# val-iisc/Reflecting-Reality

Hardware: AMD Instinct MI355X
Metric: images/sec at 512x512, 50-step DDIM, SD1.5+BrushNet (higher is better)
Workload: dtype bf16; 1 GPU; SD1.5 + BrushNet(6 cond ch) depth-cond inpaint, batch 4x512x512 per GPU, 50-step DDIM, CFG 7.5, VAE encode+decode included, random-init weights, inputs resident on the device; per_gpu_batch=4, global_batch=4, height=512, width=512, denoise_steps=50, parallelism=batch-shard x1 (no collective)

## Files before the change

reflecting-reality_amd/csrc/gemm_pers.hip:

```cpp
#include <hip/hip_runtime.h>

#include "gemm_conv_kernel.h"

namespace mfgemm {

namespace {

constexpr int PB_BM = 128, PB_BN = 160, PB_STAGES = 3, PB_PF = PB_STAGES - 1;
constexpr int PB_STAGE_BYTES = (PB_BM + PB_BN) * 128;
constexpr int PB_SLAB_RS = PB_BN * 2 + 16;
constexpr int PB_SLAB_OFF = PB_STAGES * PB_STAGE_BYTES;
constexpr int PB_SLAB_RST = PB_BM * 2 + 16;
constexpr int PB_SLAB_BYTES = PB_BN * PB_SLAB_RST;
static_assert(PB_SLAB_BYTES >= PB_BM * PB_SLAB_RS, "the slab region holds either layout");
constexpr int PB_LNST_OFF = PB_SLAB_OFF + PB_SLAB_BYTES;
constexpr int PB_EROW_OFF = PB_LNST_OFF + PB_BM * 8;
constexpr int PB_EROW_BYTES = 2 * PB_BN * 4;
constexpr int PB_LUT_OFF = PB_EROW_OFF + 2 * PB_EROW_BYTES;
constexpr int PB_LUT_N = 768;
constexpr int PB_SMEM = PB_LUT_OFF;
constexpr int PB_SMEM_GEGLU = PB_LUT_OFF + PB_LUT_N * 8;
static_assert(PB_SMEM_GEGLU <= 160 * 1024, "LDS");
constexpr int PB_CPR = PB_BN / 8;
constexpr int PB_CHUNKS = PB_BM * PB_CPR / 64;
constexpr int PB_CE = 6, PB_CC = 2;
static_assert(4 * PB_CE + 8 * PB_CC == PB_CHUNKS, "chunk ownership covers the slab");

template <bool F16, bool RES, bool GEGLU>
__device__ __forceinline__ void pers_item(const GemmArgs& p, int m, int n, const char* sp, const uint4& q, const char* lut) {
    const uint4 s = *reinterpret_cast<const uint4*>(sp);
    if constexpr (GEGLU) {
        float v[8], g[4];
        unpack_h8<F16>(s, v);
#pragma unroll
        for (int j = 0; j < 4; ++j) {
            const float x = v[4 + j];
            const float u = fmaf(__builtin_amdgcn_fmed3f(x, -6.0f, 5.984375f), 64.0f, 384.0f);
            const float fr = __builtin_amdgcn_fractf(u);
            const float2 e = *reinterpret_cast<const float2*>(lut + (int)(u - fr) * 8);
            g[j] = v[j] * (x * fmaf(fr, e.y, e.x));
        }
        uint2 u;
        u.x = pack_h2<F16>(g[0], g[1]);
        u.y = pack_h2<F16>(g[2], g[3]);
        *reinterpret_cast<uint2*>(p.out + ((int64_t)m * p.ldc + (n >> 1)) * 2) = u;
    } else {
        uint4 o = s;
        if (RES || p.act == MF_ACT_SILU) {
            float v[8];
            unpack_h8<F16>(s, v);
            if constexpr (RES) {
                float r[8];
                unpack_h8<F16>(q, r);
#pragma unroll
                for (int j = 0; j < 8; ++j) v[j] += r[j];
            }
            if (p.act == MF_ACT_SILU) {
#pragma unroll
                for (int j = 0; j < 8; ++j) v[j] = silu_precise(v[j]);
            }
            o = pack_h8<F16>(v);
        }
        *reinterpret_cast<uint4*>(p.out + ((int64_t)m * p.ldc + n) * 2) = o;
    }
}

__device__ __forceinline__ void pers_item_vt(const GemmArgs& p, int m, int n, const char* sp) {
    const uint4 s = *reinterpret_cast<const uint4*>(sp);
    const int img = m / p.vt_tokens, tok = m - img * p.vt_tokens;
    *reinterpret_cast<uint4*>(p.vt_out + (((int64_t)img * (p.N - p.vt_n0) + (n - p.vt_n0)) * p.vt_ld + tok) * 2) = s;
}

template <int DT, bool RES, bool GEGLU, bool LN, bool VT>
__global__ __launch_bounds__(1024) void gemm_pers_kernel(const GemmArgs p) {
    extern __shared__ __attribute__((aligned(16))) char smem[];
    constexpr bool F16 = DT == MF_F16;
    const int tid = (int)threadIdx.x, wave = __builtin_amdgcn_readfirstlane(tid >> 6), lane = tid & 63;
    const int role = wave < 8 ? 0 : (wave < 12 ? 1 : 2), rw = role == 0 ? wave : (wave & 3);
    int bid = (int)blockIdx.x;
    {
        const int nblk = (int)gridDim.x, q = nblk >> 3, r = nblk & 7, x = bid & 7, j = bid >> 3;
        bid = (x < r ? x * (q + 1) : r * (q + 1) + (x - r) * q) + j;
    }
    const int range = bid / p.tiles_m, tile_m = bid - range * p.tiles_m;
    const int m0 = tile_m * PB_BM, nt0 = range * p.nloop;
    const int nkt = p.nkt, G = p.nloop * nkt;
    const unsigned lds0 = __builtin_amdgcn_readfirstlane((unsigned)(size_t)(lds_ptr_t)smem);
    float2* lnst = reinterpret_cast<float2*>(smem + PB_LNST_OFF);
    const int dbg = p.dbg_epi;

    if constexpr (GEGLU) {
        if (tid < PB_LUT_N) {
            const float x0 = -6.0f + (float)tid * 0.015625f, x1 = x0 + 0.015625f;
            const float p0 = 0.5f * erfcf(-x0 * 0.70710678118654752440f), p1 = 0.5f * erfcf(-x1 * 0.70710678118654752440f);
            *reinterpret_cast<float2*>(smem + PB_LUT_OFF + tid * 8) = make_float2(p0, p1 - p0);
        }
        __builtin_amdgcn_s_waitcnt(0xc07f);
    }

    auto item_coords = [&](int c, int& row, int& cg) {
        int it = c * 64 + lane;
        asm volatile("" : "+v"(it));
        row = it / PB_CPR;
        cg = it - row * PB_CPR;
    };
    auto do_chunk = [&](int c, int n0, const uint4& qv) {
        if (VT && n0 >= p.vt_n0) {
            int it = c * 64 + lane;
            asm volatile("" : "+v"(it));
            const int col = it >> 4, rg = it & 15;
            pers_item_vt(p, m0 + rg * 8, n0 + col, smem + PB_SLAB_OFF + col * PB_SLAB_RST + rg * 16);
            return;
        }
        int row, cg;
        item_coords(c, row, cg);
        uint4 q = qv;
        if constexpr (RES) asm volatile("" : "+v"(q.x), "+v"(q.y), "+v"(q.z), "+v"(q.w));
        pers_item<F16, RES, GEGLU>(p, m0 + row, n0 + cg * 8, smem + PB_SLAB_OFF + row * PB_SLAB_RS + cg * 16, q, smem + PB_LUT_OFF);
    };
    auto fetch_res = [&](int c, int n0) -> uint4 {
        int row, cg;
        item_coords(c, row, cg);
        return *reinterpret_cast<const uint4*>(p.res0 + ((int64_t)(m0 + row) * p.ld_res0 + n0 + cg * 8) * 2);
    };

    if ((GEGLU || (dbg & 16)) && role == 0) __builtin_amdgcn_s_setprio(1);
    if ((dbg & 32) && role == 1) __builtin_amdgcn_s_setprio(1);
    if ((dbg & 64) && role == 2) __builtin_amdgcn_s_setprio(1);
    if (role == 1) {
        const srd_t sA = make_srd(p.a0, (unsigned)((int64_t)p.M * p.ld0b));
        const srd_t sW = make_srd(p.w, (unsigned)(((int64_t)(p.N - 1) * p.ldw + p.K) * 2));
        const int r8 = lane >> 3, slot = lane & 7;
        unsigned offA[4], offW[5];
#pragma unroll
        for (int i = 0; i < 4; ++i) {
            const int r = (4 * rw + i) * 8 + r8;
            offA[i] = (unsigned)(m0 + r) * (unsigned)p.ld0b + (unsigned)((slot ^ ((r >> 1) & 7)) << 4);
        }
#pragma unroll
        for (int i = 0; i < 5; ++i) {
            const int r = (5 * rw + i) * 8 + r8;
            offW[i] = (unsigned)(nt0 * PB_BN + r) * (unsigned)(p.ldw * 2) + (unsigned)((slot ^ ((r >> 1) & 7)) << 4);
        }
        const unsigned wstep = (unsigned)PB_BN * (unsigned)(p.ldw * 2);
        int i_kt = 0, i_st = 0;
        unsigned wbase = 0;
        const bool nodma = (dbg & 4) != 0;
        auto issue = [&]() {
            const unsigned ldsS = lds0 + i_st * PB_STAGE_BYTES;
            if (!nodma) {
#pragma unroll
                for (int i = 0; i < 4; ++i) dma16_buf(offA[i] + i_kt * 128, sA, ldsS + ((4 * rw + i) * 8) * 128);
#pragma unroll
                for (int i = 0; i < 5; ++i) dma16_buf(offW[i] + wbase + i_kt * 128, sW, ldsS + PB_BM * 128 + ((5 * rw + i) * 8) * 128);
            }
            i_st = i_st == PB_STAGES - 1 ? 0 : i_st + 1;
            if (++i_kt == nkt) { i_kt = 0; wbase += wstep; }
        };
        auto wait_newer = [&](int newer) {
            if (newer >= 2) wait_vmcnt<18>();
            else if (newer == 1) wait_vmcnt<9>();
            else wait_vmcnt<0>();
        };
        static_assert(PB_PF <= 2, "wait_newer covers 0 .. 2 younger tiles");
        for (int k = 0; k < PB_PF && k < G; ++k) issue();
        wait_newer((G < PB_PF ? G : PB_PF) - 1);
        __builtin_amdgcn_s_barrier();
        for (int g = 0; g + 1 < G; ++g) {
            if (g + PB_PF < G) issue();
            const int youngest = g + PB_PF < G ? g + PB_PF : G - 1;
            wait_newer(youngest - (g + 1));
            __builtin_amdgcn_s_barrier();
        }
        __builtin_amdgcn_s_barrier();
    } else if (role == 0) {
        const int wm = rw >> 1, wn = rw & 1, r16 = lane & 15, kg = lane >> 4;
        const int key16 = (r16 >> 1) & 7;
        f32x4_t acc[2][5];
#pragma unroll
        for (int a = 0; a < 2; ++a)
#pragma unroll
            for (int b = 0; b < 5; ++b) acc[a][b] = f32x4_t{0.0f, 0.0f, 0.0f, 0.0f};
        auto dump_vt = [&](int jt) {
            const char* er = smem + PB_EROW_OFF + (jt & 1) * PB_EROW_BYTES;
            const float alpha = p.alpha;
            const int odd = r16 & 1;
            float2 rst[2];
            if constexpr (LN) {
#pragma unroll
                for (int a = 0; a < 2; ++a) rst[a] = lnst[wm * 32 + 16 * a + r16];
            }
#pragma unroll
            for (int b = 0; b < 5; ++b) {
                const int col = wn * 80 + 16 * b + 4 * kg;
                const float4 bias = *reinterpret_cast<const float4*>(er + col * 4);
                float4 cs = make_float4(0, 0, 0, 0);
                if constexpr (LN) cs = *reinterpret_cast<const float4*>(er + PB_BN * 4 + col * 4);
#pragma unroll
                for (int a = 0; a < 2; ++a) {
                    float x[4] = {acc[a][b][0], acc[a][b][1], acc[a][b][2], acc[a][b][3]};
                    if constexpr (LN) {
                        x[0] = rst[a].y * (x[0] - rst[a].x * cs.x); x[1] = rst[a].y * (x[1] - rst[a].x * cs.y);
                        x[2] = rst[a].y * (x[2] - rst[a].x * cs.z); x[3] = rst[a].y * (x[3] - rst[a].x * cs.w);
                    }
                    x[0] = (x[0] + bias.x) * alpha; x[1] = (x[1] + bias.y) * alpha; x[2] = (x[2] + bias.z) * alpha; x[3] = (x[3] + bias.w) * alpha;
                    const float s0 = odd ? x[0] : x[2], s1 = odd ? x[1] : x[3];
                    const float g0 = __builtin_bit_cast(float, __builtin_amdgcn_mov_dpp(__builtin_bit_cast(int, s0), 0xB1, 0xF, 0xF, true));
                    const float g1 = __builtin_bit_cast(float, __builtin_amdgcn_mov_dpp(__builtin_bit_cast(int, s1), 0xB1, 0xF, 0xF, true));
                    const uint32_t d0 = pack_h2<F16>(odd ? g0 : x[0], odd ? x[2] : g0);
                    const uint32_t d1 = pack_h2<F16>(odd ? g1 : x[1], odd ? x[3] : g1);
                    char* sp = smem + PB_SLAB_OFF + (col + 2 * odd) * PB_SLAB_RST + (wm * 32 + 16 * a + (r16 & ~1)) * 2;
                    *reinterpret_cast<uint32_t*>(sp) = d0;
                    *reinterpret_cast<uint32_t*>(sp + PB_SLAB_RST) = d1;
                    acc[a][b] = f32x4_t{0.0f, 0.0f, 0.0f, 0.0f};
                }
            }
        };
        auto dump_plain = [&](int jt) {
            const char* er = smem + PB_EROW_OFF + (jt & 1) * PB_EROW_BYTES;
            const float alpha = p.alpha;
            float2 rst[2];
            if constexpr (LN) {
#pragma unroll
                for (int a = 0; a < 2; ++a) rst[a] = lnst[wm * 32 + 16 * a + r16];
            }
#pragma unroll
            for (int b = 0; b < 5; ++b) {
                const int col = wn * 80 + 16 * b + 4 * kg;
                const float4 bias = *reinterpret_cast<const float4*>(er + col * 4);
                float4 cs = make_float4(0, 0, 0, 0);
                if constexpr (LN) cs = *reinterpret_cast<const float4*>(er + PB_BN * 4 + col * 4);
#pragma unroll
                for (int a = 0; a < 2; ++a) {
                    float x[4] = {acc[a][b][0], acc[a][b][1], acc[a][b][2], acc[a][b][3]};
                    if constexpr (LN) {
                        x[0] = rst[a].y * (x[0] - rst[a].x * cs.x); x[1] = rst[a].y * (x[1] - rst[a].x * cs.y);
                        x[2] = rst[a].y * (x[2] - rst[a].x * cs.z); x[3] = rst[a].y * (x[3] - rst[a].x * cs.w);
                    }
                    x[0] = (x[0] + bias.x) * alpha; x[1] = (x[1] + bias.y) * alpha; x[2] = (x[2] + bias.z) * alpha; x[3] = (x[3] + bias.w) * alpha;
                    uint2 h;
                    h.x = pack_h2<F16>(x[0], x[1]);
                    h.y = pack_h2<F16>(x[2], x[3]);
                    *reinterpret_cast<uint2*>(smem + PB_SLAB_OFF + (wm * 32 + 16 * a + r16) * PB_SLAB_RS + col * 2) = h;
                    acc[a][b] = f32x4_t{0.0f, 0.0f, 0.0f, 0.0f};
                }
            }
        };
        auto is_vt = [&](int jt) -> bool { return VT && (nt0 + jt) * PB_BN >= p.vt_n0; };
        auto dump = [&](int jt) {
            if (is_vt(jt)) dump_vt(jt);
            else dump_plain(jt);
        };
        uint4 q[RES ? PB_CC : 1];
        auto prefetch = [&](int jt) {
            if constexpr (RES) {
                const int n0 = (nt0 + jt) * PB_BN;
#pragma unroll
                for (int i = 0; i < PB_CC; ++i) q[i] = fetch_res(4 * PB_CE + PB_CC * rw + i, n0);
            }
        };
        if (p.nloop > 1) prefetch(0);
        const int avail = nkt - 1, per = (PB_CC + avail - 1) / avail;
        int st = 0, kt = 0, jt = 0, pend_n0 = -1, done = 0;
        const bool nomma = (dbg & 2) != 0;
        __builtin_amdgcn_s_barrier();
        for (int g = 0; g < G; ++g) {
            const bool dumping = kt == 0 && g > 0;
            if (dumping && !(dbg & 8)) dump(jt - 1);
            if (!nomma) {
                const char* A16 = smem + st * PB_STAGE_BYTES + (wm * 32 + r16) * 128;
                const char* B16 = smem + st * PB_STAGE_BYTES + PB_BM * 128 + (wn * 80 + r16) * 128;
                uint4 fa[2][2], fb[2][5];
#pragma unroll
                for (int ks = 0; ks < 2; ++ks) {
#pragma unroll
                    for (int a = 0; a < 2; ++a) fa[ks][a] = *reinterpret_cast<const uint4*>(A16 + a * 16 * 128 + (((4 * ks + kg) ^ key16) << 4));
#pragma unroll
                    for (int b = 0; b < 5; ++b) fb[ks][b] = *reinterpret_cast<const uint4*>(B16 + b * 16 * 128 + (((4 * ks + kg) ^ key16) << 4));
                }
#pragma unroll
                for (int ks = 0; ks < 2; ++ks)
#pragma unroll
                    for (int a = 0; a < 2; ++a)
#pragma unroll
                        for (int b = 0; b < 5; ++b)
                            acc[a][b] = mfma16x32<DT>(__builtin_bit_cast(bf16x8_t, fb[ks][b]), __builtin_bit_cast(bf16x8_t, fa[ks][a]), acc[a][b], 0, 0, 0);
            }
            st = st == PB_STAGES - 1 ? 0 : st + 1;
            if (pend_n0 >= 0 && !dumping) {
                if (done == 0) {
                    if constexpr (RES) {
                        asm volatile("s_waitcnt vmcnt(0)" ::: "memory");
#pragma unroll
                        for (int i = 0; i < PB_CC; ++i) asm volatile("" : "+v"(q[i].x), "+v"(q[i].y), "+v"(q[i].z), "+v"(q[i].w));
                    }
                }
#pragma unroll 1
                for (int i = 0; i < per && done < PB_CC; ++i, ++done) {
                    if (dbg & 1) continue;
                    if (done == 0) do_chunk(4 * PB_CE + PB_CC * rw, pend_n0, q[0]);
                    else do_chunk(4 * PB_CE + PB_CC * rw + 1, pend_n0, q[RES ? 1 : 0]);
                }
                if (done == PB_CC) {
                    pend_n0 = -1;
                    if (jt < p.nloop - 1) prefetch(jt);
                }
            }
            if (dumping) { pend_n0 = (nt0 + jt - 1) * PB_BN; done = 0; }
            if (++kt == nkt) { kt = 0; ++jt; }
            __builtin_amdgcn_s_waitcnt(0xc07f);
            __builtin_amdgcn_s_barrier();
        }
        dump(p.nloop - 1);
        __builtin_amdgcn_s_waitcnt(0xc07f);
    } else {
        uint4 q[RES ? PB_CE : 1];
        float4 pb = make_float4(0, 0, 0, 0), pc = make_float4(0, 0, 0, 0);
        constexpr bool rows_duty = true;
        auto prefetch = [&](int jt) {
            if constexpr (RES) {
                const int n0 = (nt0 + jt) * PB_BN;
#pragma unroll
                for (int i = 0; i < PB_CE; ++i) q[i] = fetch_res(PB_CE * rw + i, n0);
            }
        };
        const float* brow = p.bias ? p.bias : reinterpret_cast<const float*>(p.w);
        const int rlane = lane < PB_BN / 4 ? lane : lane - PB_BN / 4;
        auto fetch_rows = [&](int jt) {
            const int n0 = (nt0 + jt) * PB_BN;
            pb = *reinterpret_cast<const float4*>(brow + n0 + rlane * 4);
            if constexpr (LN) pc = *reinterpret_cast<const float4*>(p.ln_cs + n0 + rlane * 4);
        };
        auto publish_rows = [&](int jt) {
            if (rw == 0 && lane < PB_BN / 4) {
                char* er = smem + PB_EROW_OFF + (jt & 1) * PB_EROW_BYTES;
                *reinterpret_cast<float4*>(er + lane * 16) = p.bias ? pb : make_float4(0, 0, 0, 0);
                *reinterpret_cast<float4*>(er + PB_BN * 4 + lane * 16) = pc;
            }
        };
        fetch_rows(0);
        asm volatile("s_waitcnt vmcnt(0)" ::: "memory");
        publish_rows(0);
        if (p.nloop > 1) {
            fetch_rows(1);
            asm volatile("s_waitcnt vmcnt(0)" ::: "memory");
            publish_rows(1);
            prefetch(0);
        }
        fetch_rows(p.nloop > 2 ? 2 : p.nloop - 1);
        float ls1 = 0.0f, ls2 = 0.0f;
        const int lrow = rw * 32 + (lane >> 1), lhalf = lane & 1;
        const int avail = nkt - 1, per = (PB_CE + avail - 1) / avail;
        int pend_n0 = -1, pend_jt = 0, done = 0, kt = 0, jt = 0, st = 0;
        __builtin_amdgcn_s_waitcnt(0xc07f);
        __builtin_amdgcn_s_barrier();
        for (int g = 0; g < G; ++g) {
            if (LN && g < nkt) {
                const char* ar = smem + st * PB_STAGE_BYTES + lrow * 128 + lhalf * 64;
#pragma unroll
                for (int c = 0; c < 4; ++c) {
                    float x[8];
                    unpack_h8<F16>(*reinterpret_cast<const uint4*>(ar + c * 16), x);
#pragma unroll
                    for (int e = 0; e < 8; ++e) { ls1 += x[e]; ls2 = fmaf(x[e], x[e], ls2); }
                }
                if (g == nkt - 1) {
                    ls1 += __shfl_xor(ls1, 1); ls2 += __shfl_xor(ls2, 1);
                    const float invk = 1.0f / (float)p.K, mean = ls1 * invk;
                    float var = ls2 * invk - mean * mean;
                    if (var < 0.0f) var = 0.0f;
                    if (lhalf == 0) lnst[lrow] = make_float2(mean, 1.0f / sqrtf(var + p.ln_eps));
                }
            }
            st = st == PB_STAGES - 1 ? 0 : st + 1;
            if (pend_n0 >= 0) {
                if (done == 0) {
                    if (RES || rows_duty) asm volatile("s_waitcnt vmcnt(0)" ::: "memory");
                    if constexpr (RES) {
#pragma unroll
                        for (int i = 0; i < PB_CE; ++i) asm volatile("" : "+v"(q[i].x), "+v"(q[i].y), "+v"(q[i].z), "+v"(q[i].w));
                    }
                    asm volatile("" : "+v"(pb.x), "+v"(pb.y), "+v"(pb.z), "+v"(pb.w), "+v"(pc.x), "+v"(pc.y), "+v"(pc.z), "+v"(pc.w));
                    if (pend_jt + 2 < p.nloop) publish_rows(pend_jt + 2);
                    fetch_rows(pend_jt + 3 < p.nloop ? pend_jt + 3 : p.nloop - 1);
                }
#pragma unroll 1
                for (int i = 0; i < per && done < PB_CE; ++i, ++done) {
                    if (dbg & 1) continue;
                    switch (done) {
                        case 0: do_chunk(PB_CE * rw + 0, pend_n0, q[0]); break;
                        case 1: do_chunk(PB_CE * rw + 1, pend_n0, q[RES ? 1 : 0]); break;
                        case 2: do_chunk(PB_CE * rw + 2, pend_n0, q[RES ? 2 : 0]); break;
                        case 3: do_chunk(PB_CE * rw + 3, pend_n0, q[RES ? 3 : 0]); break;
                        case 4: do_chunk(PB_CE * rw + 4, pend_n0, q[RES ? 4 : 0]); break;
                        default: do_chunk(PB_CE * rw + 5, pend_n0, q[RES ? 5 : 0]); break;
                    }
                }
                if (done == PB_CE) {
                    pend_n0 = -1;
                    if (pend_jt + 1 < p.nloop - 1) prefetch(pend_jt + 1);
                }
            }
            __builtin_amdgcn_s_waitcnt(0xc07f);
            __builtin_amdgcn_s_barrier();
            if (kt == 0 && jt > 0) { pend_n0 = (nt0 + jt - 1) * PB_BN; pend_jt = jt - 1; done = 0; }
            if (++kt == nkt) { kt = 0; ++jt; }
        }
    }
    __builtin_amdgcn_s_barrier();
    {
        const int n0 = (nt0 + p.nloop - 1) * PB_BN;
        for (int c = wave; c < PB_CHUNKS; c += 16) {
            if (VT && n0 >= p.vt_n0) {
                if (!(dbg & 1)) do_chunk(c, n0, uint4{0, 0, 0, 0});
                continue;
            }
            int row, cg;
            item_coords(c, row, cg);
            uint4 q = uint4{0, 0, 0, 0};
            if constexpr (RES) q = *reinterpret_cast<const uint4*>(p.res0 + ((int64_t)(m0 + row) * p.ld_res0 + n0 + cg * 8) * 2);
            if (!(dbg & 1)) pers_item<F16, RES, GEGLU>(p, m0 + row, n0 + cg * 8, smem + PB_SLAB_OFF + row * PB_SLAB_RS + cg * 16, q, smem + PB_LUT_OFF);
        }
    }
}

}

template <int DT>
static const void* pers_fn(bool res, bool geglu, bool ln, bool vt) {
    if (vt) return ln ? reinterpret_cast<const void*>(&gemm_pers_kernel<DT, false, false, true, true>) : reinterpret_cast<const void*>(&gemm_pers_kernel<DT, false, false, false, true>);
    if (geglu) return ln ? reinterpret_cast<const void*>(&gemm_pers_kernel<DT, false, true, true, false>) : reinterpret_cast<const void*>(&gemm_pers_kernel<DT, false, true, false, false>);
    if (res) return ln ? reinterpret_cast<const void*>(&gemm_pers_kernel<DT, true, false, true, false>) : reinterpret_cast<const void*>(&gemm_pers_kernel<DT, true, false, false, false>);
    return ln ? reinterpret_cast<const void*>(&gemm_pers_kernel<DT, false, false, true, false>) : reinterpret_cast<const void*>(&gemm_pers_kernel<DT, false, false, false, false>);
}

bool launch_pers(int dtype, const GemmArgs& a, hipStream_t s) {
    if (dtype != MF_BF16 && dtype != MF_F16) return false;
    const bool geglu = a.act == MF_ACT_GEGLU4, res = a.res0 != nullptr, ln = a.ln_cs != nullptr, vt = a.vt_out != nullptr;
    if ((geglu && res) || (vt && (geglu || res))) return false;
    const int fl = dtype == MF_F16 ? 1 : 0, variant = (vt ? 6 : geglu ? 4 : (res ? 2 : 0)) + (ln ? 1 : 0);
    const void* fn = fl ? pers_fn<MF_F16>(res, geglu, ln, vt) : pers_fn<MF_BF16>(res, geglu, ln, vt);
    static bool attr[2][8][64] = {};
    int dev = 0;
    if (hipGetDevice(&dev) != hipSuccess || dev < 0 || dev >= 64) return false;
    if (!attr[fl][variant][dev]) {
        if (hipFuncSetAttribute(fn, hipFuncAttributeMaxDynamicSharedMemorySize, PB_SMEM_GEGLU) != hipSuccess) return false;
        attr[fl][variant][dev] = true;
    }
    void* args[] = {const_cast<GemmArgs*>(&a)};
    return hipLaunchKernel(fn, dim3((unsigned)(a.tiles_m * (a.tiles_n / a.nloop))), dim3(1024), args, geglu ? PB_SMEM_GEGLU : PB_SMEM, s) == hipSuccess;
}

}
```

Baseline: 5.268 images/sec.

## Restructure persistent GEMM role loops into nested tile/k loops with precomputed offsets

Rewrites the producer, MFMA and epilogue wave loops of the persistent GEMM as nested jt/kt loops instead of one flat loop with running counters. DMA and LDS fragment addresses are precomputed and advanced incrementally, and the producer gets a fixed vmcnt(9) steady-state wait. MFMA and LDS reads are interleaved through sched_group_barrier hints, and epilogue chunks are scheduled at fixed k-intervals. The goal is less scalar/VALU bookkeeping and better instruction interleaving in the inner loop. It also adds optional clock-stamp instrumentation behind MF_STAMPS, at the cost of more complex control flow and tighter static assumptions.

```diff
diff --git a/reflecting-reality_amd/csrc/gemm_pers.hip b/reflecting-reality_amd/csrc/gemm_pers.hip
--- a/reflecting-reality_amd/csrc/gemm_pers.hip
+++ b/reflecting-reality_amd/csrc/gemm_pers.hip
@@ -1,6 +1,18 @@
 #include <hip/hip_runtime.h>
 
 #include "gemm_conv_kernel.h"
+
+#ifdef MF_STAMPS
+#define PB_CLOCKS() unsigned long long pb_work = 0, pb_wait = 0, pb_n = 0, pb_rel = __builtin_amdgcn_s_memtime()
+#define PB_BARRIER() do { const unsigned long long a_ = __builtin_amdgcn_s_memtime(); __builtin_amdgcn_s_barrier(); \
+    const unsigned long long r_ = __builtin_amdgcn_s_memtime(); pb_work += a_ - pb_rel; pb_wait += r_ - a_; ++pb_n; pb_rel = r_; } while (0)
+#define PB_CLOCKS_PUT() do { if (p.stamps && rw == 0 && lane == 0) { unsigned long long* s_ = p.stamps + (size_t)blockIdx.x * 32 + 8 * role; \
+    s_[0] = pb_work; s_[1] = pb_wait; s_[3] = pb_n; } } while (0)
+#else
+#define PB_CLOCKS() do { } while (0)
+#define PB_BARRIER() __builtin_amdgcn_s_barrier()
+#define PB_CLOCKS_PUT() do { } while (0)
+#endif
 
 namespace mfgemm {
 
@@ -143,19 +155,20 @@
             offW[i] = (unsigned)(nt0 * PB_BN + r) * (unsigned)(p.ldw * 2) + (unsigned)((slot ^ ((r >> 1) & 7)) << 4);
         }
         const unsigned wstep = (unsigned)PB_BN * (unsigned)(p.ldw * 2);
-        int i_kt = 0, i_st = 0;
-        unsigned wbase = 0;
+        const unsigned ldsA0 = lds0 + (unsigned)(4 * rw * 8 * 128), ldsW = (unsigned)(PB_BM * 128 + (5 * rw - 4 * rw) * 8 * 128);
+        const unsigned kend = (unsigned)nkt * 128u;
+        unsigned koff = 0, woff = 0, ldsA = ldsA0;
         const bool nodma = (dbg & 4) != 0;
         auto issue = [&]() {
-            const unsigned ldsS = lds0 + i_st * PB_STAGE_BYTES;
-            if (!nodma) {
-#pragma unroll
-                for (int i = 0; i < 4; ++i) dma16_buf(offA[i] + i_kt * 128, sA, ldsS + ((4 * rw + i) * 8) * 128);
-#pragma unroll
-                for (int i = 0; i < 5; ++i) dma16_buf(offW[i] + wbase + i_kt * 128, sW, ldsS + PB_BM * 128 + ((5 * rw + i) * 8) * 128);
-            }
-            i_st = i_st == PB_STAGES - 1 ? 0 : i_st + 1;
-            if (++i_kt == nkt) { i_kt = 0; wbase += wstep; }
+            if (__builtin_expect(!nodma, 1)) {
+#pragma unroll
+                for (int i = 0; i < 4; ++i) dma16_buf(offA[i] + koff, sA, ldsA + i * 8 * 128);
+#pragma unroll
+                for (int i = 0; i < 5; ++i) dma16_buf(offW[i] + woff, sW, ldsA + ldsW + i * 8 * 128);
+            }
+            ldsA = ldsA == ldsA0 + (PB_STAGES - 1) * PB_STAGE_BYTES ? ldsA0 : ldsA + PB_STAGE_BYTES;
+            koff += 128; woff += 128;
+            if (koff == kend) { koff = 0; woff += wstep - kend; }
         };
         auto wait_newer = [&](int newer) {
             if (newer >= 2) wait_vmcnt<18>();
@@ -166,12 +179,18 @@
         for (int k = 0; k < PB_PF && k < G; ++k) issue();
         wait_newer((G < PB_PF ? G : PB_PF) - 1);
         __builtin_amdgcn_s_barrier();
-        for (int g = 0; g + 1 < G; ++g) {
-            if (g + PB_PF < G) issue();
-            const int youngest = g + PB_PF < G ? g + PB_PF : G - 1;
-            wait_newer(youngest - (g + 1));
-            __builtin_amdgcn_s_barrier();
-        }
+        PB_CLOCKS();
+        static_assert(PB_PF == 2, "the steady-state wait below leaves one tile (nine DMAs) in flight");
+        for (int g = 0; g + PB_PF < G; ++g) {
+            issue();
+            wait_vmcnt<9>();
+            PB_BARRIER();
+        }
+        if (G >= PB_PF) {
+            wait_vmcnt<0>();
+            PB_BARRIER();
+        }
+        PB_CLOCKS_PUT();
         __builtin_amdgcn_s_barrier();
     } else if (role == 0) {
         const int wm = rw >> 1, wn = rw & 1, r16 = lane & 15, kg = lane >> 4;
@@ -259,24 +278,34 @@
                 for (int i = 0; i < PB_CC; ++i) q[i] = fetch_res(4 * PB_CE + PB_CC * rw + i, n0);
             }
         };
-        if (p.nloop > 1) prefetch(0);
-        const int avail = nkt - 1, per = (PB_CC + avail - 1) / avail;
-        int st = 0, kt = 0, jt = 0, pend_n0 = -1, done = 0;
-        const bool nomma = (dbg & 2) != 0;
+        const int nloop = p.nloop;
+        if (nloop > 1) prefetch(0);
+        const int avail = nkt - 1, per = (PB_CC + avail - 1) / avail, last_ci = (PB_CC + per - 1) / per;
+        static_assert(PB_CC == 2, "one chunk in interval 1, the other in interval last_ci");
+        const bool nomma = (dbg & 2) != 0, nochunk = (dbg & 1) != 0, nodump = (dbg & 8) != 0;
+        unsigned fo[4];
+        {
+            const unsigned laneA = (unsigned)((wm * 32 + r16) * 128), laneB = (unsigned)(PB_BM * 128 + (wn * 80 + r16) * 128);
+            const unsigned sw0 = (unsigned)((kg ^ key16) << 4), sw1 = (unsigned)(((4 + kg) ^ key16) << 4);
+            fo[0] = lds0 + laneA + sw0; fo[1] = lds0 + laneA + sw1; fo[2] = lds0 + laneB + sw0; fo[3] = lds0 + laneB + sw1;
+        }
+        typedef unsigned int u32x4_t __attribute__((ext_vector_type(4)));
+        typedef __attribute__((address_space(3))) const u32x4_t* lds_q4_t;
+        int st = 0;
         __builtin_amdgcn_s_barrier();
-        for (int g = 0; g < G; ++g) {
-            const bool dumping = kt == 0 && g > 0;
-            if (dumping && !(dbg & 8)) dump(jt - 1);
-            if (!nomma) {
-                const char* A16 = smem + st * PB_STAGE_BYTES + (wm * 32 + r16) * 128;
-                const char* B16 = smem + st * PB_STAGE_BYTES + PB_BM * 128 + (wn * 80 + r16) * 128;
+        PB_CLOCKS();
+        for (int jt = 0; jt < nloop; ++jt) {
+          const int pend_n0 = (nt0 + jt - 1) * PB_BN;
+          for (int kt = 0; kt < nkt; ++kt) {
+            if (kt == 0 && jt > 0 && !nodump) dump(jt - 1);
+            if (__builtin_expect(!nomma, 1)) {
                 uint4 fa[2][2], fb[2][5];
 #pragma unroll
                 for (int ks = 0; ks < 2; ++ks) {
 #pragma unroll
-                    for (int a = 0; a < 2; ++a) fa[ks][a] = *reinterpret_cast<const uint4*>(A16 + a * 16 * 128 + (((4 * ks + kg) ^ key16) << 4));
-#pragma unroll
-                    for (int b = 0; b < 5; ++b) fb[ks][b] = *reinterpret_cast<const uint4*>(B16 + b * 16 * 128 + (((4 * ks + kg) ^ key16) << 4));
+                    for (int a = 0; a < 2; ++a) fa[ks][a] = __builtin_bit_cast(uint4, *(lds_q4_t)(size_t)(fo[ks] + a * 16 * 128));
+#pragma unroll
+                    for (int b = 0; b < 5; ++b) fb[ks][b] = __builtin_bit_cast(uint4, *(lds_q4_t)(size_t)(fo[2 + ks] + b * 16 * 128));
                 }
 #pragma unroll
                 for (int ks = 0; ks < 2; ++ks)
@@ -285,33 +314,40 @@
 #pragma unroll
                         for (int b = 0; b < 5; ++b)
                             acc[a][b] = mfma16x32<DT>(__builtin_bit_cast(bf16x8_t, fb[ks][b]), __builtin_bit_cast(bf16x8_t, fa[ks][a]), acc[a][b], 0, 0, 0);
-            }
-            st = st == PB_STAGES - 1 ? 0 : st + 1;
-            if (pend_n0 >= 0 && !dumping) {
-                if (done == 0) {
+                __builtin_amdgcn_sched_group_barrier(0x100, 7, 0);
+#pragma unroll
+                for (int i = 0; i < 7; ++i) {
+                    __builtin_amdgcn_sched_group_barrier(0x008, 1, 0);
+                    __builtin_amdgcn_sched_group_barrier(0x100, 1, 0);
+                }
+                __builtin_amdgcn_sched_group_barrier(0x008, 13, 0);
+            }
+            if (jt > 0 && kt >= 1 && kt <= last_ci) {
+                if (kt == 1) {
                     if constexpr (RES) {
                         asm volatile("s_waitcnt vmcnt(0)" ::: "memory");
 #pragma unroll
                         for (int i = 0; i < PB_CC; ++i) asm volatile("" : "+v"(q[i].x), "+v"(q[i].y), "+v"(q[i].z), "+v"(q[i].w));
                     }
                 }
-#pragma unroll 1
-                for (int i = 0; i < per && done < PB_CC; ++i, ++done) {
-                    if (dbg & 1) continue;
-                    if (done == 0) do_chunk(4 * PB_CE + PB_CC * rw, pend_n0, q[0]);
-                    else do_chunk(4 * PB_CE + PB_CC * rw + 1, pend_n0, q[RES ? 1 : 0]);
-                }
-                if (done == PB_CC) {
-                    pend_n0 = -1;
-                    if (jt < p.nloop - 1) prefetch(jt);
-                }
-            }
-            if (dumping) { pend_n0 = (nt0 + jt - 1) * PB_BN; done = 0; }
-            if (++kt == nkt) { kt = 0; ++jt; }
+                if (!nochunk) {
+                    if (kt == 1) do_chunk(4 * PB_CE + PB_CC * rw, pend_n0, q[0]);
+                    if (kt == last_ci) do_chunk(4 * PB_CE + PB_CC * rw + 1, pend_n0, q[RES ? 1 : 0]);
+                }
+                if (kt == last_ci && jt < nloop - 1) prefetch(jt);
+            }
+            {
+                const unsigned step = st == PB_STAGES - 1 ? 0u - (PB_STAGES - 1) * PB_STAGE_BYTES : (unsigned)PB_STAGE_BYTES;
+                st = st == PB_STAGES - 1 ? 0 : st + 1;
+#pragma unroll
+                for (int i = 0; i < 4; ++i) { fo[i] += step; asm volatile("" : "+v"(fo[i])); }
+            }
             __builtin_amdgcn_s_waitcnt(0xc07f);
-            __builtin_amdgcn_s_barrier();
-        }
-        dump(p.nloop - 1);
+            PB_BARRIER();
+          }
+        }
+        PB_CLOCKS_PUT();
+        dump(nloop - 1);
         __builtin_amdgcn_s_waitcnt(0xc07f);
     } else {
         uint4 q[RES ? PB_CE : 1];
@@ -350,13 +386,19 @@
         fetch_rows(p.nloop > 2 ? 2 : p.nloop - 1);
         float ls1 = 0.0f, ls2 = 0.0f;
         const int lrow = rw * 32 + (lane >> 1), lhalf = lane & 1;
-        const int avail = nkt - 1, per = (PB_CE + avail - 1) / avail;
-        int pend_n0 = -1, pend_jt = 0, done = 0, kt = 0, jt = 0, st = 0;
+        const int nloop = p.nloop;
+        const int avail = nkt - 1, per = (PB_CE + avail - 1) / avail, last_ci = (PB_CE + per - 1) / per;
+        const bool nochunk = (dbg & 1) != 0;
+        [[maybe_unused]] int lst = 0;
         __builtin_amdgcn_s_waitcnt(0xc07f);
         __builtin_amdgcn_s_barrier();
-        for (int g = 0; g < G; ++g) {
-            if (LN && g < nkt) {
-                const char* ar = smem + st * PB_STAGE_BYTES + lrow * 128 + lhalf * 64;
+        PB_CLOCKS();
+        for (int jt = 0; jt < nloop; ++jt) {
+          const int pend_n0 = (nt0 + jt - 1) * PB_BN;
+          for (int kt = 0; kt < nkt; ++kt) {
+            if (LN && jt == 0) {
+                const char* ar = smem + lst * PB_STAGE_BYTES + lrow * 128 + lhalf * 64;
+                lst = lst == PB_STAGES - 1 ? 0 : lst + 1;
 #pragma unroll
                 for (int c = 0; c < 4; ++c) {
                     float x[8];
@@ -364,7 +406,7 @@
 #pragma unroll
                     for (int e = 0; e < 8; ++e) { ls1 += x[e]; ls2 = fmaf(x[e], x[e], ls2); }
                 }
-                if (g == nkt - 1) {
+                if (kt == nkt - 1) {
                     ls1 += __shfl_xor(ls1, 1); ls2 += __shfl_xor(ls2, 1);
                     const float invk = 1.0f / (float)p.K, mean = ls1 * invk;
                     float var = ls2 * invk - mean * mean;
@@ -372,40 +414,30 @@
                     if (lhalf == 0) lnst[lrow] = make_float2(mean, 1.0f / sqrtf(var + p.ln_eps));
                 }
             }
-            st = st == PB_STAGES - 1 ? 0 : st + 1;
-            if (pend_n0 >= 0) {
-                if (done == 0) {
+            if (jt > 0 && kt >= 1 && kt <= last_ci) {
+                if (kt == 1) {
                     if (RES || rows_duty) asm volatile("s_waitcnt vmcnt(0)" ::: "memory");
                     if constexpr (RES) {
 #pragma unroll
                         for (int i = 0; i < PB_CE; ++i) asm volatile("" : "+v"(q[i].x), "+v"(q[i].y), "+v"(q[i].z), "+v"(q[i].w));
                     }
                     asm volatile("" : "+v"(pb.x), "+v"(pb.y), "+v"(pb.z), "+v"(pb.w), "+v"(pc.x), "+v"(pc.y), "+v"(pc.z), "+v"(pc.w));
-                    if (pend_jt + 2 < p.nloop) publish_rows(pend_jt + 2);
-                    fetch_rows(pend_jt + 3 < p.nloop ? pend_jt + 3 : p.nloop - 1);
-                }
-#pragma unroll 1
-                for (int i = 0; i < per && done < PB_CE; ++i, ++done) {
-                    if (dbg & 1) continue;
-                    switch (done) {
-                        case 0: do_chunk(PB_CE * rw + 0, pend_n0, q[0]); break;
-                        case 1: do_chunk(PB_CE * rw + 1, pend_n0, q[RES ? 1 : 0]); break;
-                        case 2: do_chunk(PB_CE * rw + 2, pend_n0, q[RES ? 2 : 0]); break;
-                        case 3: do_chunk(PB_CE * rw + 3, pend_n0, q[RES ? 3 : 0]); break;
-                        case 4: do_chunk(PB_CE * rw + 4, pend_n0, q[RES ? 4 : 0]); break;
-                        default: do_chunk(PB_CE * rw + 5, pend_n0, q[RES ? 5 : 0]); break;
-                    }
-                }
-                if (done == PB_CE) {
-                    pend_n0 = -1;
-                    if (pend_jt + 1 < p.nloop - 1) prefetch(pend_jt + 1);
-                }
+                    if (jt + 1 < nloop) publish_rows(jt + 1);
+                    fetch_rows(jt + 2 < nloop ? jt + 2 : nloop - 1);
+                }
+                if (!nochunk) {
+                    const int c0 = (kt - 1) * per, c1 = c0 + per;
+#pragma unroll
+                    for (int c = 0; c < PB_CE; ++c)
+                        if (c >= c0 && c < c1) do_chunk(PB_CE * rw + c, pend_n0, q[RES ? c : 0]);
+                }
+                if (kt == last_ci && jt < nloop - 1) prefetch(jt);
             }
             __builtin_amdgcn_s_waitcnt(0xc07f);
-            __builtin_amdgcn_s_barrier();
-            if (kt == 0 && jt > 0) { pend_n0 = (nt0 + jt - 1) * PB_BN; pend_jt = jt - 1; done = 0; }
-            if (++kt == nkt) { kt = 0; ++jt; }
-        }
+            PB_BARRIER();
+          }
+        }
+        PB_CLOCKS_PUT();
     }
     __builtin_amdgcn_s_barrier();
     {
```

Measured after the change: 5.266 images/sec. No clear change (-0.0%).
